# IlzeAmandaA/VAE-GP-ODE

Hardware: AMD Instinct MI355X
Metric: latent_trajectories_per_sec (higher is better)
Workload: dtype f32; 1 GPU; configs[1]: ode1 DF q=6 M=100 S=256 T=16 batch=256; step = full ELBO training step (encoder, GP draw, rk4 rollout, decoder, ELBO, backward, Adam), L=1; global_batch=256, mc_draws=1, solver=rk4 (3/8 rule), parallelism=dp1, hip_graph=True, graph_scope=whole, gp_side_stream=True, batchnorm=per-process statistics

## Files before the change

vae-gp-ode_amd/csrc/gp_backward.hip:

```cpp
#include "gp_rollout.hpp"

namespace gp {

template <int DI, int DO, int NJ>
__device__ __forceinline__ void store_grads_rbf(const typename RbfTeamEval<DI, DO, NJ>::Grads& G, float* __restrict__ out, int M, int S,
                                                int wave, int lane, float (*sInd)[64][4 * RbfLayout<DI, DO>::RQ2],
                                                float (*sUni)[((DO + 1) / 2) * DI]);
template <int D, int NJ, int PART = 0>
__device__ __forceinline__ void store_grads_df(const typename DfTeamEval<D, NJ>::Grads& G, float* __restrict__ out, int M, int S, int wave,
                                               int lane, float (*sInd)[64][4 * DfLayout<D>::RQ2],
                                               float (*sUni)[2 * D * ((D + 1) / 2) + (D + 1) / 2]);

template <class EV, bool PG> struct GradsOf { using type = NoGrads; };
template <class EV> struct GradsOf<EV, true> { using type = typename EV::Grads; };

template <class EV, int DI, int DO, int ORDER, int METHOD, bool PG = false, bool SUB = false>
__global__ __launch_bounds__(64 * EV::kTeam) void rollout_bwd_team_kernel(const float* __restrict__ pack, int M, int S,
                                                                const float* __restrict__ xstage, const float* __restrict__ gzt,
                                                                const float* __restrict__ ts, int N, int T,
                                                                float* __restrict__ gz0, float* __restrict__ astage, Draws dw,
                                                                float* __restrict__ slab = nullptr, size_t pack_floats = 0) {
  constexpr int NS = stages_of(METHOD);
  __shared__ float slots[2 * EV::kTeam * TeamCombine::DP];
  pack += blockIdx.y * dw.pack; xstage += blockIdx.y * dw.in; gzt += blockIdx.y * dw.in2; gz0 += blockIdx.y * dw.out; astage += blockIdx.y * dw.out2;
// ... 87 lines not shown
    } else {
      using L = DfLayout<DO>;
      constexpr int DH = (DO + 1) / 2;
      __shared__ __attribute__((aligned(16))) float sInd[2][64][4 * L::RQ2];
      __shared__ float sUni[TEAM][2 * DO * DH + DH];
      store_grads_df<DO, 1>(G, out, M, S, wave, lane, sInd, sUni);
    }
  }
}

template <class EV, int DI, int DO>
__global__ __launch_bounds__(64 * EV::kTeam) void rhs_vjp_team_kernel(const float* __restrict__ pack, int M, int S,
                                                            const float* __restrict__ x, const float* __restrict__ a, int R,
                                                            float* __restrict__ gx, int prior_only, Draws dw) {
  __shared__ float slots[2 * EV::kTeam * TeamCombine::DP];
  pack += blockIdx.y * dw.pack; x += blockIdx.y * dw.in; a += blockIdx.y * dw.in2; gx += blockIdx.y * dw.out;
  const int lane = threadIdx.x & 63, wave = threadIdx.x >> 6;
  EV ev;
  ev.init(pack, M, S, slots, wave, lane);
  for (int n = blockIdx.x; n < R; n += gridDim.x) {
    float xv[DI], av[DO], g[DI];
#pragma unroll
    for (int i = 0; i < DI; ++i) xv[i] = x[(size_t)n * DI + i];
#pragma unroll
    for (int i = 0; i < DO; ++i) av[i] = a[(size_t)n * DO + i];
    ev.vjp(xv, av, g, prior_only != 0);
    if (wave == 0) store_state<DI>(gx + (size_t)n * DI, g, lane);
  }
}

__device__ __forceinline__ void st4(float* __restrict__ base, size_t f4_index, const float* v) {
  reinterpret_cast<float4*>(base)[f4_index] = make_float4(v[0], v[1], v[2], v[3]);
}

template <int DI, int DO, int NJ>
__device__ __forceinline__ void store_grads_rbf(const typename RbfTeamEval<DI, DO, NJ>::Grads& G, float* __restrict__ out, int M, int S,
                                                int wave, int lane, float (*sInd)[64][4 * RbfLayout<DI, DO>::RQ2],
                                                float (*sUni)[((DO + 1) / 2) * DI]) {
  using L = RbfLayout<DI, DO>;
  constexpr int DH = (DO + 1) / 2;
  const int SJ = cdiv(S, 64), MJ = cdiv(M, 64);
#pragma unroll
  for (int jn = 0; jn < NJ; ++jn) {
    const int j = wave + TEAM * jn;
    if (j < SJ) {
#pragma unroll
      for (int d = 0; d < DO; ++d)
#pragma unroll
        for (int q = 0; q < L::RQ; ++q) st4(out, (size_t)((j * DO + d) * L::RQ + q) * 64 + lane, &G.rff[jn * DO + d][4 * q]);
    }
  }
  const int j = wave >> 1, half = wave & 1;
  if (half == 1) {
#pragma unroll
    for (int q = 0; q < 4 * L::RQ2; ++q) sInd[j][lane][q] = G.ind[q];
  }
  {
    float flat[DH * DI], red[DH * DI];
#pragma unroll
    for (int e = 0; e < DH * DI; ++e) flat[e] = G.gwl[e / DI][e % DI];
    wave_sum_all<DH * DI>(flat, red);
    if (lane == 0) {
#pragma unroll
      for (int e = 0; e < DH * DI; ++e) sUni[wave][e] = red[e];
    }
  }
  __syncthreads();
  if (half == 0 && j < MJ) {
    float* ind_out = out + 4 * L::rff_f4(S);
    float v[4 * L::RQ2];
#pragma unroll
    for (int q = 0; q < 4 * L::RQ2; ++q) v[q] = G.ind[q] + sInd[j][lane][q];
#pragma unroll
    for (int q = 0; q < L::RQ2; ++q) st4(ind_out, (size_t)(j * L::RQ2 + q) * 64 + lane, &v[4 * q]);
  }
  if (threadIdx.x < DO * DI) {
    const int d = threadIdx.x / DI, i = threadIdx.x % DI;
    const int h = d / DH, dd = d % DH;
    float* uni_out = out + 4 * (L::rff_f4(S) + L::ind_f4(M));
    uni_out[d * DI + i] = sUni[h][dd * DI + i] + sUni[h + 2][dd * DI + i];
  }
}

template <int DI, int DO, int NJ>
__global__ __launch_bounds__(256) void param_grad_rbf_kernel(const float* __restrict__ pack, int M, int S,
                                                              const float* __restrict__ xr, const float* __restrict__ ar,
                                                              int R, int rows_per_chunk, float* __restrict__ slab,
                                                              size_t pack_floats, int prior_only, Draws dw, int slab_chunks) {
  pack += blockIdx.y * dw.pack; xr += blockIdx.y * dw.in; ar += blockIdx.y * dw.in2; slab += (size_t)blockIdx.y * slab_chunks * pack_floats;
  using EV = RbfTeamEval<DI, DO, NJ>;
  using L = RbfLayout<DI, DO>;
  constexpr int DH = (DO + 1) / 2;
  __shared__ float slots[2 * TEAM * TeamCombine::DP];
  __shared__ __attribute__((aligned(16))) float sInd[2][64][4 * L::RQ2];
  __shared__ float sUni[TEAM][DH * DI];
  const int lane = threadIdx.x & 63, wave = threadIdx.x >> 6;
  EV ev;
  ev.init(pack, M, S, slots, wave, lane);
  typename EV::Grads G;
  G.zero();
  const int r0 = blockIdx.x * rows_per_chunk;
  const int r1 = min(R, r0 + rows_per_chunk);
  for (int r = r0; r < r1; ++r) {
    float x[DI], a[DO];
#pragma unroll
    for (int i = 0; i < DI; ++i) x[i] = xr[(size_t)r * DI + i];
#pragma unroll
    for (int i = 0; i < DO; ++i) a[i] = ar[(size_t)r * DO + i];
    ev.grad_row(x, a, G, prior_only != 0);
  }
  store_grads_rbf<DI, DO, NJ>(G, slab + (size_t)blockIdx.x * pack_floats, M, S, wave, lane, sInd, sUni);
}

template <int D, int NJ, int PART>
__device__ __forceinline__ void store_grads_df(const typename DfTeamEval<D, NJ>::Grads& G, float* __restrict__ out, int M, int S, int wave,
                                               int lane, float (*sInd)[64][4 * DfLayout<D>::RQ2],
                                               float (*sUni)[2 * D * ((D + 1) / 2) + (D + 1) / 2]) {
  using L = DfLayout<D>;
  constexpr int DH = (D + 1) / 2;
  constexpr int NU = 2 * D * DH + DH;
  const int SJ = cdiv(S, 64), MJ = cdiv(M, 64);
  if constexpr (PART != 2) {
#pragma unroll
    for (int jn = 0; jn < NJ; ++jn) {
      const int j = wave + TEAM * jn;
      if (j < SJ) {
#pragma unroll
        for (int i = 0; i < D; ++i)
#pragma unroll
          for (int q = 0; q < L::RQ; ++q) st4(out, (size_t)((j * D + i) * L::RQ + q) * 64 + lane, &G.rff[jn * D + i][4 * q]);
      }
    }
  }
  if constexpr (PART == 1) return;
  const int j = wave >> 1, half = wave & 1;
  if (half == 1) {
#pragma unroll
    for (int q = 0; q < 4 * L::RQ2; ++q) sInd[j][lane][q] = G.ind[q];
  }
  {
    float flat[NU];
#pragma unroll
    for (int a = 0; a < D; ++a)
#pragma unroll
      for (int b = 0; b < DH; ++b) { flat[a * DH + b] = G.gwab[a][b]; flat[D * DH + a * DH + b] = G.gil2[a][b]; }
#pragma unroll
    for (int b = 0; b < DH; ++b) flat[2 * D * DH + b] = G.gvar[b];
    float red[NU];
    wave_sum_all<NU>(flat, red);
    if (lane == 0) {
#pragma unroll
      for (int e = 0; e < NU; ++e) sUni[wave][e] = red[e];
    }
  }
  __syncthreads();
  if (half == 0 && j < MJ) {
    float* ind_out = out + 4 * L::rff_f4(S);
    float v[4 * L::RQ2];
#pragma unroll
    for (int q = 0; q < 4 * L::RQ2; ++q) v[q] = G.ind[q] + sInd[j][lane][q];
#pragma unroll
    for (int q = 0; q < L::RQ2; ++q) st4(ind_out, (size_t)(j * L::RQ2 + q) * 64 + lane, &v[4 * q]);
  }
  {
    float* uni_out = out + 4 * (L::rff_f4(S) + L::ind_f4(M));
    const int t = threadIdx.x;
    if (t < D * D) {
      const int a = t / D, b = t % D, h = b / DH, bb = b % DH;
      uni_out[a * D + b] = sUni[h][a * DH + bb] + sUni[h + 2][a * DH + bb];
      uni_out[D * D + a * D + b] = sUni[h][D * DH + a * DH + bb] + sUni[h + 2][D * DH + a * DH + bb];
    }
    if (t < D) {
      const int h = t / DH, bb = t % DH;
      uni_out[2 * D * D + t] = sUni[h][2 * D * DH + bb] + sUni[h + 2][2 * D * DH + bb];
    }
  }
}

template <int D, int NJ>
__global__ __launch_bounds__(256) void param_grad_df_kernel(const float* __restrict__ pack, int M, int S,
                                                             const float* __restrict__ xr, const float* __restrict__ ar,
                                                             int R, int rows_per_chunk, float* __restrict__ slab,
                                                             size_t pack_floats, int prior_only, Draws dw, int slab_chunks) {
  pack += blockIdx.y * dw.pack; xr += blockIdx.y * dw.in; ar += blockIdx.y * dw.in2; slab += (size_t)blockIdx.y * slab_chunks * pack_floats;
  using EV = DfTeamEval<D, NJ>;
  using L = DfLayout<D>;
  constexpr int DH = (D + 1) / 2;
  constexpr int NU = 2 * D * DH + DH;
  __shared__ float slots[2 * TEAM * TeamCombine::DP];
  __shared__ __attribute__((aligned(16))) float sInd[2][64][4 * L::RQ2];
  __shared__ float sUni[TEAM][NU];
  const int lane = threadIdx.x & 63, wave = threadIdx.x >> 6;
  EV ev;
  ev.init(pack, M, S, slots, wave, lane);
  typename EV::Grads G;
  G.zero();
  const int r0 = blockIdx.x * rows_per_chunk;
  const int r1 = min(R, r0 + rows_per_chunk);
  for (int r = r0; r < r1; ++r) {
    float x[D], a[D];
#pragma unroll
    for (int i = 0; i < D; ++i) { x[i] = xr[(size_t)r * D + i]; a[i] = ar[(size_t)r * D + i]; }
    ev.grad_row(x, a, G, prior_only != 0);
  }
  store_grads_df<D, NJ>(G, slab + (size_t)blockIdx.x * pack_floats, M, S, wave, lane, sInd, sUni);
}

template <int D, int PART>
__device__ __forceinline__ void pgrad_df_part(const float* __restrict__ pack, int M, int S, const float* __restrict__ xr,
                                              const float* __restrict__ ar, int r0, int r1, float* __restrict__ out, int prior_only) {
  using EV = DfTeamEval<D, 1>;
  using L = DfLayout<D>;
  constexpr int DH = (D + 1) / 2;
  constexpr int NU = 2 * D * DH + DH;
  __shared__ float slots[2 * TEAM * TeamCombine::DP];
  __shared__ __attribute__((aligned(16))) float sInd[2][64][4 * L::RQ2];
  __shared__ float sUni[TEAM][NU];
  const int lane = threadIdx.x & 63, wave = threadIdx.x >> 6;
  EV ev;
  ev.init(pack, M, S, slots, wave, lane);
  typename EV::Grads G;
  G.zero();
  for (int r = r0; r < r1; ++r) {
    float x[D], a[D];
#pragma unroll
    for (int i = 0; i < D; ++i) { x[i] = xr[(size_t)r * D + i]; a[i] = ar[(size_t)r * D + i]; }
    ev.template grad_row_part<PART>(x, a, G, prior_only != 0);
  }
  store_grads_df<D, 1, PART>(G, out, M, S, wave, lane, sInd, sUni);
}
template <int D>
__global__ __launch_bounds__(256, 2) void param_grad_df_split_kernel(const float* __restrict__ pack, int M, int S,
                                                                      const float* __restrict__ xr, const float* __restrict__ ar,
                                                                      int R, int rows_per_chunk, float* __restrict__ slab,
                                                                      size_t pack_floats, int prior_only, Draws dw, int slab_chunks) {
  pack += blockIdx.y * dw.pack; xr += blockIdx.y * dw.in; ar += blockIdx.y * dw.in2; slab += (size_t)blockIdx.y * slab_chunks * pack_floats;
  const int r0 = blockIdx.x * rows_per_chunk, r1 = min(R, r0 + rows_per_chunk);
  float* out = slab + (size_t)blockIdx.x * pack_floats;
  if (blockIdx.z == 0) pgrad_df_part<D, 1>(pack, M, S, xr, ar, r0, r1, out, prior_only);
  else pgrad_df_part<D, 2>(pack, M, S, xr, ar, r0, r1, out, prior_only);
}

template <int DI, int DO>
__global__ __launch_bounds__(256) void param_grad_rbf_stream_kernel(const float* __restrict__ pack, int M, int S,
                                                                     const float* __restrict__ xr, const float* __restrict__ ar,
                                                                     int R, int rows_per_chunk, float* __restrict__ slab,
                                                                     size_t pack_floats, int prior_only, Draws dw, int slab_chunks) {
  pack += blockIdx.y * dw.pack; xr += blockIdx.y * dw.in; ar += blockIdx.y * dw.in2; slab += (size_t)blockIdx.y * slab_chunks * pack_floats;
  using L = RbfLayout<DI, DO>;
  constexpr int DH = (DO + 1) / 2;
  __shared__ __attribute__((aligned(16))) float sInd[2][64][4 * L::RQ2];
  __shared__ float sUni[TEAM][DH * DI];
  const int lane = threadIdx.x & 63, wave = __builtin_amdgcn_readfirstlane(threadIdx.x >> 6);
  const float4* p4 = reinterpret_cast<const float4*>(pack);
  const float4* i4 = p4 + L::rff_f4(S);
  const float* wl = pack + 4 * (L::rff_f4(S) + L::ind_f4(M));
  const int r0 = blockIdx.x * rows_per_chunk, r1 = min(R, r0 + rows_per_chunk);
  float* out = slab + (size_t)blockIdx.x * pack_floats;
  const int SJ = cdiv(S, 64), MJ = cdiv(M, 64);
  for (int rec = wave; rec < SJ * DO; rec += TEAM) {
    float4 rq[L::RQ];
    load_record<L::RQ>(p4, rec, lane, rq);
    float g[4 * L::RQ];
#pragma unroll
    for (int q = 0; q < 4 * L::RQ; ++q) g[q] = 0.f;
    const int d = rec % DO;
    for (int r = r0; r < r1; ++r) {
      float x[DI], gx[DI];
#pragma unroll
      for (int i = 0; i < DI; ++i) { x[i] = xr[(size_t)r * DI + i]; gx[i] = 0.f; }
      rbf_rff_bwd<DI, DO, true>(rq, x, ar[(size_t)r * DO + d], gx, g);
    }
#pragma unroll
    for (int q = 0; q < L::RQ; ++q) st4(out, ((size_t)rec * L::RQ + q) * 64 + lane, &g[4 * q]);
  }
  const int half = wave & 1;
  float gwl[DH][DI];
#pragma unroll
  for (int d = 0; d < DH; ++d)
#pragma unroll
    for (int i = 0; i < DI; ++i) gwl[d][i] = 0.f;
  float* ind_out = out + 4 * L::rff_f4(S);
  for (int jb = 0; jb < MJ; jb += 2) {
    const int j = jb + (wave >> 1);
    const bool valid = j < MJ;
    float4 ind[L::RQ2];
    float gi[4 * L::RQ2];
#pragma unroll
    for (int q = 0; q < 4 * L::RQ2; ++q) gi[q] = 0.f;
    if (valid) {
      load_record<L::RQ2>(i4, j, lane, ind);
      if (!prior_only) {
        for (int r = r0; r < r1; ++r) {
          asm volatile("" ::: "memory");
          float x[DI], a[DO], gx[DI];
#pragma unroll
          for (int i = 0; i < DI; ++i) { x[i] = xr[(size_t)r * DI + i]; gx[i] = 0.f; }
#pragma unroll
          for (int i = 0; i < DO; ++i) a[i] = ar[(size_t)r * DO + i];
          rbf_ind_half_bwd<DI, DO, true>(ind, x, wl, half, a, gx, gi, gwl);
        }
      }
    }
    if (half == 1) {
#pragma unroll
      for (int q = 0; q < 4 * L::RQ2; ++q) sInd[wave >> 1][lane][q] = gi[q];
    }
    __syncthreads();
    if (half == 0 && valid) {
      float v[4 * L::RQ2];
#pragma unroll
// ... 306 lines not shown
```

vae-gp-ode_amd/csrc/gp_eval.hpp:

```cpp
#pragma once
#include <hip/hip_runtime.h>
#include "wave_reduce.hpp"

#define GP_WAVE 64
#define GP_LOG2E 1.4426950408889634f
#define GP_INV2PI 0.15915494309189535f

namespace gp {

__host__ __device__ constexpr int cdiv(int a, int b) { return (a + b - 1) / b; }

template <int DI, int DO> struct RbfLayout {
  static constexpr int RQ = cdiv(DI + 2, 4);
  static constexpr int RQ2 = cdiv(DI + DO, 4);
  __host__ __device__ static size_t rff_f4(int S) { return (size_t)cdiv(S, 64) * DO * RQ * 64; }
  __host__ __device__ static size_t ind_f4(int M) { return (size_t)cdiv(M, 64) * RQ2 * 64; }
  __host__ __device__ static size_t uni_floats() { return (size_t)cdiv(DO * DI, 4) * 4; }
  __host__ __device__ static size_t total_floats(int M, int S) { return 4 * (rff_f4(S) + ind_f4(M)) + uni_floats(); }
};

template <int D> struct DfLayout {
  static constexpr int RQ = cdiv(2 * D + 3, 4);
  static constexpr int RQ2 = cdiv(2 * D, 4);
  __host__ __device__ static size_t rff_f4(int S) { return (size_t)cdiv(S, 64) * D * RQ * 64; }
// ... 220 lines not shown
#pragma unroll
  for (int k = 0; k < D; ++k) t = fmaf(x[k], f[k], t);
  t = __builtin_amdgcn_fractf(t);
  const float c = __builtin_amdgcn_cosf(t), sn = __builtin_amdgcn_sinf(t);
  float A = 0.f;
#pragma unroll
  for (int j = 0; j < D; ++j) A = fmaf(a[j], f[D + 3 + j], A);
  const float rt = GP_2PI * fmaf(f[D + 2], c, -f[D + 1] * sn);
  const float coef = A * rt;
#pragma unroll
  for (int k = 0; k < D; ++k) gx[k] = fmaf(coef, f[k], gx[k]);
  if (WITH_G) {
    const float rr = fmaf(f[D + 2], sn, f[D + 1] * c);
#pragma unroll
    for (int k = 0; k < D; ++k) g[k] = fmaf(coef, x[k], g[k]);
#pragma unroll
    for (int j = 0; j < D; ++j) g[D + 3 + j] = fmaf(a[j], rr, g[D + 3 + j]);
  }
}

template <int D, bool WITH_G>
__device__ __forceinline__ void df_ind_half_bwd(const float4 (&r)[DfLayout<D>::RQ2], const float (&x)[D],
                                                const float* __restrict__ uni, int half, const float (&a)[D],
                                                float (&gx)[D], float (&g)[4 * DfLayout<D>::RQ2],
                                                float (&gwab)[D][(D + 1) / 2], float (&gil2)[D][(D + 1) / 2],
                                                float (&gvar)[(D + 1) / 2]) {
  constexpr int DH = (D + 1) / 2;
  float f[4 * DfLayout<D>::RQ2];
  unpack(r, f);
  const float* wab = uni;
  const float* il2 = uni + D * D;
  const float* var = uni + 2 * D * D;
  float dl[D];
  float r2 = 0.f;
#pragma unroll
  for (int q = 0; q < D; ++q) { dl[q] = x[q] - f[q]; r2 = fmaf(dl[q], dl[q], r2); }
  const int b0 = half * DH;
  float gd[D];
  float gr2 = 0.f;
#pragma unroll
  for (int q = 0; q < D; ++q) gd[q] = 0.f;
#pragma unroll
  for (int bb = 0; bb < DH; ++bb) {
    const bool hi_ok = DH + bb < D;
    const int bidx = b0 + bb < D ? b0 + bb : D - 1;
    const bool live = half ? hi_ok : true;
    const float dlb = half ? (hi_ok ? dl[hi_ok ? DH + bb : 0] : 0.f) : dl[bb];
    const float ab = live ? (half ? (hi_ok ? a[hi_ok ? DH + bb : 0] : 0.f) : a[bb]) : 0.f;
    const float vb = var[bidx];
    float gdb = 0.f;
    float gv = 0.f;
#pragma unroll
    for (int aa = 0; aa < D; ++aa) {
      const float il = il2[aa * D + bidx], wv = wab[aa * D + bidx];
      const float E = exp2_fast(r2 * wv);
      const bool diag = (aa == bidx);
      const float term = dl[aa] * dlb * il + (diag ? ((float)(D - 1) - r2 * il) : 0.f);
      const float G = ab * f[D + aa];
      const float GE = G * vb * E * il;
      gr2 = fmaf(GE, term * (GP_LN2 * wv) - (diag ? il : 0.f), gr2);
      gd[aa] = fmaf(GE * il, dlb, gd[aa]);
      gdb = fmaf(GE * il, dl[aa], gdb);
      if (WITH_G) {
        g[D + aa] = fmaf(ab, vb * E * il * term, g[D + aa]);
        gv = fmaf(G, E * il * term, gv);
        gwab[aa][bb] = fmaf(G * vb * il * term, E * GP_LN2 * r2, gwab[aa][bb]);
        gil2[aa][bb] = fmaf(G * vb * E, term + il * (dl[aa] * dlb - (diag ? r2 : 0.f)), gil2[aa][bb]);
      }
    }
    if (WITH_G) gvar[bb] += gv;
    if (live) {
      if (half) { if (hi_ok) gd[hi_ok ? DH + bb : 0] += gdb; }
      else gd[bb] += gdb;
    }
  }
#pragma unroll
  for (int q = 0; q < D; ++q) {
    const float v = fmaf(2.f * gr2, dl[q], gd[q]);
    gx[q] += v;
    if (WITH_G) g[q] -= v;
  }
}

template <int DI, int DO>
__device__ __forceinline__ void rbf_rff_jvp(const float4 (&r)[RbfLayout<DI, DO>::RQ], const float (&x)[DI], const float (&v)[DI],
                                            float& acc, float& jacc) {
  float f[4 * RbfLayout<DI, DO>::RQ];
  unpack(r, f);
  float t = f[DI], tv = 0.f;
#pragma unroll
  for (int i = 0; i < DI; ++i) { t = fmaf(x[i], f[i], t); tv = fmaf(v[i], f[i], tv); }
  t = __builtin_amdgcn_fractf(t);
  const float c = __builtin_amdgcn_cosf(t), sn = __builtin_amdgcn_sinf(t);
  acc = fmaf(f[DI + 1], c, acc);
  jacc = fmaf(f[DI + 1] * (-GP_2PI) * sn, tv, jacc);
}

template <int DI, int DO>
__device__ __forceinline__ void rbf_ind_jvp(const float4 (&r)[RbfLayout<DI, DO>::RQ2], const float (&x)[DI], const float (&v)[DI],
                                            const float* __restrict__ wl, float (&acc)[DO], float (&jacc)[DO]) {
  float f[4 * RbfLayout<DI, DO>::RQ2];
  unpack(r, f);
  float t2[DI], dt2[DI];
#pragma unroll
  for (int i = 0; i < DI; ++i) { const float d = x[i] - f[i]; t2[i] = d * d; dt2[i] = 2.f * d * v[i]; }
#pragma unroll
  for (int d = 0; d < DO; ++d) {
    float e = 0.f, de = 0.f;
#pragma unroll
    for (int i = 0; i < DI; ++i) { e = fmaf(wl[d * DI + i], t2[i], e); de = fmaf(wl[d * DI + i], dt2[i], de); }
    const float E = exp2_fast(e);
    acc[d] = fmaf(f[DI + d], E, acc[d]);
    jacc[d] = fmaf(f[DI + d] * E, GP_LN2 * de, jacc[d]);
  }
}

template <int D>
__device__ __forceinline__ void df_rff_jvp(const float4 (&r)[DfLayout<D>::RQ], const float (&x)[D], const float (&v)[D],
                                           float (&acc)[D], float (&jacc)[D]) {
  float f[4 * DfLayout<D>::RQ];
  unpack(r, f);
  float t = f[D], tv = 0.f;
#pragma unroll
  for (int k = 0; k < D; ++k) { t = fmaf(x[k], f[k], t); tv = fmaf(v[k], f[k], tv); }
  t = __builtin_amdgcn_fractf(t);
  const float c = __builtin_amdgcn_cosf(t), sn = __builtin_amdgcn_sinf(t);
  const float rr = fmaf(f[D + 2], sn, f[D + 1] * c);
  const float drr = GP_2PI * fmaf(f[D + 2], c, -f[D + 1] * sn) * tv;
#pragma unroll
  for (int j = 0; j < D; ++j) { acc[j] = fmaf(rr, f[D + 3 + j], acc[j]); jacc[j] = fmaf(drr, f[D + 3 + j], jacc[j]); }
}

template <int D>
__device__ __forceinline__ void df_ind_jvp(const float4 (&r)[DfLayout<D>::RQ2], const float (&x)[D], const float (&v)[D],
                                           const float* __restrict__ uni, float (&acc)[D], float (&jacc)[D]) {
  float f[4 * DfLayout<D>::RQ2];
  unpack(r, f);
  const float* wab = uni;
  const float* il2 = uni + D * D;
  const float* var = uni + 2 * D * D;
  float dl[D];
  float r2 = 0.f, dr2 = 0.f;
#pragma unroll
  for (int a = 0; a < D; ++a) { dl[a] = x[a] - f[a]; r2 = fmaf(dl[a], dl[a], r2); dr2 = fmaf(dl[a], v[a], dr2); }
  dr2 *= 2.f;
  if constexpr (D > 8) {
    constexpr int DH = (D + 1) / 2;
#pragma unroll 1
    for (int half = 0; half < 2; ++half) {
#pragma unroll
      for (int bb = 0; bb < DH; ++bb) {
        const bool valid = DH + bb < D;
        const int bidx = half * DH + bb < D ? half * DH + bb : D - 1;
        const float dlb = half ? (valid ? dl[valid ? DH + bb : 0] : 0.f) : dl[bb];
        const float vb = half ? (valid ? v[valid ? DH + bb : 0] : 0.f) : v[bb];
        float sb = 0.f, dsb = 0.f;
#pragma unroll
        for (int a = 0; a < D; ++a) {
          const float il = il2[a * D + bidx], wv = wab[a * D + bidx];
          const float E = exp2_fast(r2 * wv);
          const bool diag = (a == bidx);
          const float term = dl[a] * dlb * il + (diag ? ((float)(D - 1) - r2 * il) : 0.f);
          const float dterm = fmaf(v[a], dlb, dl[a] * vb) * il - (diag ? dr2 * il : 0.f);
          const float cf = f[D + a] * (E * il);
          sb = fmaf(cf, term, sb);
          dsb = fmaf(cf, fmaf(term, GP_LN2 * wv * dr2, dterm), dsb);
// ... 30 lines not shown
```

vae-gp-ode_amd/csrc/gp_team.hpp:

```cpp
#pragma once
#include "gp_eval.hpp"

namespace gp {

constexpr int TEAM = 4;

template <int TS> struct TeamCombineT {
  static constexpr int DP = 16;
  float* slots;
  int wave, lane, parity;
  __device__ __forceinline__ void init(float* s, int w, int l) { slots = s; wave = w; lane = l; parity = 0; }
  template <int NV> __device__ __forceinline__ void run(const float (&part)[NV], float (&f)[NV]) {
    static_assert(NV <= DP, "slot too small");
    float* mine = slots + (parity * TS + wave) * DP;
    if (lane == 0) {
#pragma unroll
      for (int d = 0; d < NV; ++d) mine[d] = part[d];
    }
    __syncthreads();
    const float* base = slots + parity * TS * DP;
#pragma unroll
    for (int d = 0; d < NV; ++d) {
      float v = base[d];
#pragma unroll
// ... 90 lines not shown
    for (int i = 0; i < DI; ++i) acc[i] = 0.f;
#pragma unroll
    for (int r = 0; r < NJ * DO; ++r) rbf_rff_bwd<DI, DO, true>(rff[r], x, a[r % DO], acc, G.rff[r]);
    rbf_ind_half_bwd<DI, DO, true>(ind, x, wl, half, a, acc, G.ind, G.gwl);
    float part[DI];
    wave_sum_all<DI>(acc, part);
    comb.run<DI>(part, gx);
  }
};

template <int D, int NJ> struct DfTeamEval {
  using L = DfLayout<D>;
  static constexpr int kTeam = TEAM;
  float4 rff[NJ * D][L::RQ];
  float4 ind[L::RQ2];
  const float* uni;
  int half;
  TeamCombine comb;
  static __host__ bool fits(int M, int S) { return cdiv(S, 64) <= TEAM * NJ && cdiv(M, 64) * 2 <= TEAM; }
  __device__ __forceinline__ void init(const float* pack, int M, int S, float* lds, int wave, int lane) {
    const float4* p4 = reinterpret_cast<const float4*>(pack);
    const int SJ = cdiv(S, 64), MJ = cdiv(M, 64);
    const float4 z = make_float4(0.f, 0.f, 0.f, 0.f);
#pragma unroll
    for (int jn = 0; jn < NJ; ++jn) {
      const int j = wave + TEAM * jn;
#pragma unroll
      for (int i = 0; i < D; ++i)
#pragma unroll
        for (int q = 0; q < L::RQ; ++q) rff[jn * D + i][q] = j < SJ ? p4[((j * D + i) * L::RQ + q) * 64 + lane] : z;
    }
    const float4* i4 = p4 + L::rff_f4(S);
    const int j = wave >> 1;
    half = wave & 1;
#pragma unroll
    for (int q = 0; q < L::RQ2; ++q) ind[q] = j < MJ ? i4[(j * L::RQ2 + q) * 64 + lane] : z;
    uni = pack + 4 * (L::rff_f4(S) + L::ind_f4(M));
    comb.init(lds, wave, lane);
  }
  template <int MODE> __device__ __forceinline__ void eval(const float (&x)[D], float (&f)[D]) {
    float acc[D];
#pragma unroll
    for (int d = 0; d < D; ++d) acc[d] = 0.f;
    if (MODE != 2) {
#pragma unroll
      for (int r = 0; r < NJ * D; ++r) df_rff_record<D>(rff[r], x, acc);
    }
    if (MODE != 1) df_ind_record_half<D>(ind, x, uni, half, acc);
    float part[D];
    wave_sum_all<D>(acc, part);
    comb.run<D>(part, f);
  }
  __device__ __forceinline__ void vjp(const float (&x)[D], const float (&a)[D], float (&gx)[D], bool prior_only = false) {
    float acc[D];
#pragma unroll
    for (int i = 0; i < D; ++i) acc[i] = 0.f;
    float g0[4 * L::RQ], g1[4 * L::RQ2], g2[D][(D + 1) / 2], g3[D][(D + 1) / 2], g4[(D + 1) / 2];
#pragma unroll
    for (int r = 0; r < NJ * D; ++r) df_rff_bwd<D, false>(rff[r], x, a, acc, g0);
    if (!prior_only) df_ind_half_bwd<D, false>(ind, x, uni, half, a, acc, g1, g2, g3, g4);
    float part[D];
    wave_sum_all<D>(acc, part);
    comb.run<D>(part, gx);
  }
  struct Grads {
    float rff[NJ * D][4 * L::RQ];
    float ind[4 * L::RQ2];
    float gwab[D][(D + 1) / 2], gil2[D][(D + 1) / 2], gvar[(D + 1) / 2];
    __device__ __forceinline__ void zero() {
#pragma unroll
      for (int r = 0; r < NJ * D; ++r)
#pragma unroll
        for (int q = 0; q < 4 * L::RQ; ++q) rff[r][q] = 0.f;
#pragma unroll
      for (int q = 0; q < 4 * L::RQ2; ++q) ind[q] = 0.f;
#pragma unroll
      for (int a = 0; a < D; ++a)
#pragma unroll
        for (int b = 0; b < (D + 1) / 2; ++b) { gwab[a][b] = 0.f; gil2[a][b] = 0.f; }
#pragma unroll
      for (int b = 0; b < (D + 1) / 2; ++b) gvar[b] = 0.f;
    }
  };
  __device__ __forceinline__ void grad_row(const float (&x)[D], const float (&a)[D], Grads& G, bool prior_only) const {
    float gx[D];
#pragma unroll
    for (int i = 0; i < D; ++i) gx[i] = 0.f;
#pragma unroll
    for (int r = 0; r < NJ * D; ++r) df_rff_bwd<D, true>(rff[r], x, a, gx, G.rff[r]);
    if (!prior_only) df_ind_half_bwd<D, true>(ind, x, uni, half, a, gx, G.ind, G.gwab, G.gil2, G.gvar);
  }
  template <int PART> __device__ __forceinline__ void grad_row_part(const float (&x)[D], const float (&a)[D], Grads& G, bool prior_only) const {
    float gx[D];
#pragma unroll
    for (int i = 0; i < D; ++i) gx[i] = 0.f;
    if constexpr (PART != 2) {
#pragma unroll
      for (int r = 0; r < NJ * D; ++r) df_rff_bwd<D, true>(rff[r], x, a, gx, G.rff[r]);
    }
    if constexpr (PART != 1) {
      if (!prior_only) df_ind_half_bwd<D, true>(ind, x, uni, half, a, gx, G.ind, G.gwab, G.gil2, G.gvar);
    }
  }
  __device__ __forceinline__ void vjp_grad(const float (&x)[D], const float (&a)[D], float (&gx)[D], Grads& G) {
    float acc[D];
#pragma unroll
    for (int i = 0; i < D; ++i) acc[i] = 0.f;
#pragma unroll
    for (int r = 0; r < NJ * D; ++r) df_rff_bwd<D, true>(rff[r], x, a, acc, G.rff[r]);
    df_ind_half_bwd<D, true>(ind, x, uni, half, a, acc, G.ind, G.gwab, G.gil2, G.gvar);
    float part[D];
    wave_sum_all<D>(acc, part);
    comb.run<D>(part, gx);
  }
};

template <int NQ>
__device__ __forceinline__ void load_record(const float4* __restrict__ base, int rec, int lane, float4 (&r)[NQ]) {
#pragma unroll
  for (int q = 0; q < NQ; ++q) r[q] = base[((size_t)rec * NQ + q) * 64 + lane];
}

template <int N> __device__ __forceinline__ float pick(const float (&v)[N], int idx) {
  float r = v[0];
#pragma unroll
  for (int i = 1; i < N; ++i) r = (idx == i) ? v[i] : r;
  return r;
}

template <int D, int NP, bool WITH_G>
__device__ __forceinline__ void df_ind_part_bwd(const float4 (&r)[DfLayout<D>::RQ2], const float (&x)[D],
                                                const float* __restrict__ uni, int part, const float (&a)[D],
                                                float (&gx)[D], float (&g)[4 * DfLayout<D>::RQ2],
                                                float (&gwab)[D][(D + NP - 1) / NP], float (&gil2)[D][(D + NP - 1) / NP],
                                                float (&gvar)[(D + NP - 1) / NP]) {
  constexpr int DQ = (D + NP - 1) / NP;
  float f[4 * DfLayout<D>::RQ2];
  unpack(r, f);
  const float* wab = uni;
  const float* il2 = uni + D * D;
  const float* var = uni + 2 * D * D;
  float dl[D];
  float r2 = 0.f;
#pragma unroll
  for (int q = 0; q < D; ++q) { dl[q] = x[q] - f[q]; r2 = fmaf(dl[q], dl[q], r2); }
  float gd[D];
  float gr2 = 0.f;
#pragma unroll
  for (int q = 0; q < D; ++q) gd[q] = 0.f;
#pragma unroll
  for (int bb = 0; bb < DQ; ++bb) {
    const int b = part * DQ + bb;
    const bool live = b < D;
    const int bidx = live ? b : D - 1;
    const float dlb = live ? pick<D>(dl, bidx) : 0.f;
    const float ab = live ? pick<D>(a, bidx) : 0.f;
    const float vb = var[bidx];
    float gdb = 0.f, gv = 0.f;
#pragma unroll
    for (int aa = 0; aa < D; ++aa) {
      const float il = il2[aa * D + bidx], wv = wab[aa * D + bidx];
      const float E = exp2_fast(r2 * wv);
      const bool diag = (aa == bidx);
      const float term = dl[aa] * dlb * il + (diag ? ((float)(D - 1) - r2 * il) : 0.f);
      const float G = ab * f[D + aa];
      const float GE = G * vb * E * il;
      gr2 = fmaf(GE, term * (GP_LN2 * wv) - (diag ? il : 0.f), gr2);
      gd[aa] = fmaf(GE * il, dlb, gd[aa]);
      gdb = fmaf(GE * il, dl[aa], gdb);
      if (WITH_G) {
        g[D + aa] = fmaf(ab, vb * E * il * term, g[D + aa]);
        gv = fmaf(G, E * il * term, gv);
        gwab[aa][bb] = fmaf(G * vb * il * term, E * GP_LN2 * r2, gwab[aa][bb]);
        gil2[aa][bb] = fmaf(G * vb * E, term + il * (dl[aa] * dlb - (diag ? r2 : 0.f)), gil2[aa][bb]);
      }
    }
    if (WITH_G) gvar[bb] += gv;
#pragma unroll
    for (int q = 0; q < D; ++q) gd[q] += (live && q == bidx) ? gdb : 0.f;
  }
#pragma unroll
  for (int q = 0; q < D; ++q) {
    const float v = fmaf(2.f * gr2, dl[q], gd[q]);
    gx[q] += v;
    if (WITH_G) g[q] -= v;
// ... 140 lines not shown
```

vae-gp-ode_amd/csrc/vae_dense.hip:

```cpp
#include <hip/hip_runtime.h>
#include "gp_launch.hpp"
#include "wave_reduce.hpp"

namespace gp {

__global__ void k_act_fwd(const float* __restrict__ x, float* __restrict__ y, size_t n, int mode) {
  for (size_t e = (size_t)blockIdx.x * blockDim.x + threadIdx.x; e < n; e += (size_t)gridDim.x * blockDim.x) {
    const float v = x[e];
    y[e] = mode == 0 ? fmaxf(v, 0.f) : 1.f / (1.f + expf(-v));
  }
}
__global__ void k_act_bwd(const float* __restrict__ y, const float* __restrict__ gy, float* __restrict__ gx, size_t n, int mode) {
  for (size_t e = (size_t)blockIdx.x * blockDim.x + threadIdx.x; e < n; e += (size_t)gridDim.x * blockDim.x) {
    const float v = y[e];
    gx[e] = mode == 0 ? (v > 0.f ? gy[e] : 0.f) : gy[e] * v * (1.f - v);
  }
}

__global__ void k_linear_fwd(const float* __restrict__ x, const float* __restrict__ w, const float* __restrict__ bias,
                             float* __restrict__ y, int B, int In, int Out) {
  const size_t e = (size_t)blockIdx.x * blockDim.x + threadIdx.x;
  if (e >= (size_t)B * Out) return;
  const int b = (int)(e / Out), o = (int)(e % Out);
  float acc = bias ? bias[o] : 0.f;
  const float* xr = x + (size_t)b * In;
  const float* wr = w + (size_t)o * In;
  for (int i = 0; i < In; ++i) acc = fmaf(xr[i], wr[i], acc);
  y[e] = acc;
}
__global__ void k_linear_bwd_x(const float* __restrict__ gy, const float* __restrict__ w, float* __restrict__ gx, int B, int In, int Out,
                               const float* __restrict__ xpre) {
  const size_t e = (size_t)blockIdx.x * blockDim.x + threadIdx.x;
  if (e >= (size_t)B * In) return;
  const int b = (int)(e / In), i = (int)(e % In);
  float acc = 0.f;
  for (int o = 0; o < Out; ++o) acc = fmaf(gy[(size_t)b * Out + o], w[(size_t)o * In + i], acc);
  gx[e] = (xpre && !(xpre[e] > 0.f)) ? 0.f : acc;
}
__global__ __launch_bounds__(256) void k_linear_bwd_w(const float* __restrict__ x, const float* __restrict__ gy, float* __restrict__ gw,
                                                       float* __restrict__ gb, int B, int In, int Out, int relu_in) {
  const int wave = (blockIdx.x * blockDim.x + threadIdx.x) >> 6, lane = threadIdx.x & 63;
  if (wave >= Out * (In + 1)) return;
  const int o = wave / (In + 1), i = wave % (In + 1);
  if (i < In ? !gw : !gb) return;
  float acc = 0.f;
  for (int b = lane; b < B; b += 64) {
    float xv = i < In ? x[(size_t)b * In + i] : 1.f;
    if (relu_in && i < In) xv = fmaxf(xv, 0.f);
    acc = fmaf(gy[(size_t)b * Out + o], xv, acc);
  }
  float in1[1] = {acc}, out1[1];
  wave_sum_multi<1>(in1, out1);
  if (lane == 0) { if (i < In) gw[(size_t)o * In + i] = out1[0]; else gb[o] = out1[0]; }
}

constexpr int LINW_SLABS = 32;
__global__ __launch_bounds__(256) void k_linear_bwd_w_cols(const float* __restrict__ x, const float* __restrict__ gy, float* __restrict__ partW,
                                                            float* __restrict__ partB, int B, int In, int Out, int rps) {
  __shared__ float red[4][9][64];
  const int lane = threadIdx.x & 63, g = threadIdx.x >> 6, o = blockIdx.x * 64 + lane;
  const int b0 = blockIdx.y * rps, b1 = min(B, b0 + rps);
  float acc[9];
#pragma unroll
  for (int i = 0; i < 9; ++i) acc[i] = 0.f;
#pragma unroll 4
  for (int b = b0 + g; b < b1; b += 4) {
    const float gv = gy[(size_t)b * Out + o];
    const float* xr = x + (size_t)b * In;
#pragma unroll
    for (int i = 0; i < 8; ++i)
      if (i < In) acc[i] = fmaf(gv, xr[i], acc[i]);
    acc[8] += gv;
  }
#pragma unroll
  for (int i = 0; i < 9; ++i) red[g][i][lane] = acc[i];
  __syncthreads();
  for (int e = threadIdx.x; e < 9 * 64; e += 256) {
    const int i = e >> 6, l = e & 63, oo = blockIdx.x * 64 + l;
    const float v = (red[0][i][l] + red[1][i][l]) + (red[2][i][l] + red[3][i][l]);
    if (i < In) partW[((size_t)blockIdx.y * Out + oo) * In + i] = v;
    else if (i == 8) partB[(size_t)blockIdx.y * Out + oo] = v;
  }
}

__global__ __launch_bounds__(256) void k_linear_fwd_fanin(const float* __restrict__ x, const float* __restrict__ w,
                                                           const float* __restrict__ bias, float* __restrict__ y, int B, int In, int Out,
                                                           int relu_in) {
  const int lane = threadIdx.x & 63;
  const int e = blockIdx.x * 4 + (threadIdx.x >> 6);
  if (e >= B * Out) return;
  const int b = e / Out, o = e % Out;
  const float* xr = x + (size_t)b * In;
  const float* wr = w + (size_t)o * In;
  float acc = 0.f;
  if (relu_in) { for (int i = lane; i < In; i += 64) acc = fmaf(fmaxf(xr[i], 0.f), wr[i], acc); }
  else { for (int i = lane; i < In; i += 64) acc = fmaf(xr[i], wr[i], acc); }
  const float in1[1] = {acc};
  float out1[1];
  wave_sum_multi<1>(in1, out1);
  if (lane == 0) y[e] = out1[0] + (bias ? bias[o] : 0.f);
}

constexpr int LIN_MAXIN = 16;
__global__ __launch_bounds__(256) void k_linear_fwd_fanout(const float* __restrict__ x, const float* __restrict__ w,
                                                            const float* __restrict__ bias, float* __restrict__ y, int B, int In, int Out,
                                                            int rows_per_block) {
  const int b0 = blockIdx.x * rows_per_block, b1 = min(B, b0 + rows_per_block);
  for (int o = blockIdx.y * 256 + threadIdx.x; o < Out; o += 256 * gridDim.y) {
    float wr[LIN_MAXIN];
#pragma unroll
    for (int i = 0; i < LIN_MAXIN; ++i) wr[i] = i < In ? w[(size_t)o * In + i] : 0.f;
    const float bo = bias ? bias[o] : 0.f;
    for (int b = b0; b < b1; ++b) {
      const float* xr = x + (size_t)b * In;
      float acc = bo;
#pragma unroll
      for (int i = 0; i < LIN_MAXIN; ++i)
        if (i < In) acc = fmaf(xr[i], wr[i], acc);
      y[(size_t)b * Out + o] = acc;
    }
  }
}
template <int OPL>
__global__ __launch_bounds__(256) void k_linear_bwd_x_fanout(const float* __restrict__ gy, const float* __restrict__ w, float* __restrict__ gx,
                                                              int B, int In) {
  const int lane = threadIdx.x & 63, wave = threadIdx.x >> 6, nw = gridDim.x * 4;
  constexpr int Out = OPL * 64;
  float wr[OPL][LIN_MAXIN];
#pragma unroll
  for (int k = 0; k < OPL; ++k)
#pragma unroll
    for (int i = 0; i < LIN_MAXIN; ++i) wr[k][i] = i < In ? w[(size_t)(lane + 64 * k) * In + i] : 0.f;
  for (int b = blockIdx.x * 4 + wave; b < B; b += nw) {
    float acc[LIN_MAXIN];
#pragma unroll
    for (int i = 0; i < LIN_MAXIN; ++i) acc[i] = 0.f;
#pragma unroll
    for (int k = 0; k < OPL; ++k) {
      const float g = gy[(size_t)b * Out + lane + 64 * k];
#pragma unroll
      for (int i = 0; i < LIN_MAXIN; ++i) acc[i] = fmaf(g, wr[k][i], acc[i]);
    }
    float tot[LIN_MAXIN];
    wave_sum_all<LIN_MAXIN>(acc, tot);
    if (lane < In) {
      float v = 0.f;
#pragma unroll
      for (int i = 0; i < LIN_MAXIN; ++i) v = (lane == i) ? tot[i] : v;
      gx[(size_t)b * In + lane] = v;
    }
  }
}

int act_fwd(const float* x, float* y, size_t n, int mode, hipStream_t st) {
  hipLaunchKernelGGL(k_act_fwd, ew_grid(n), 256, 0, st, x, y, n, mode);
// ... 68 lines not shown
```

Before: 108,700 trajectories/s.

## Prefetch GP grad rows, cache DF tail params in registers, tile linear-bwd inputs in LDS

The DF parameter-gradient kernels now prefetch the next row's x/a one iteration ahead and specialize the prior_only flag at compile time. The per-half inducing-tail hyperparameters (wab, il2, var) are loaded once into registers instead of being re-read from the uniform pack on every row. Separately, the linear-layer weight-gradient kernel stages input rows in shared memory per 128-row tile and batches its gy loads. The changes are meant to hide global-load latency and cut redundant loads, at the cost of extra registers, which may lower occupancy.

```diff
diff --git a/vae-gp-ode_amd/csrc/gp_backward.hip b/vae-gp-ode_amd/csrc/gp_backward.hip
--- a/vae-gp-ode_amd/csrc/gp_backward.hip
+++ b/vae-gp-ode_amd/csrc/gp_backward.hip
@@ -193,6 +193,37 @@
   }
 }
 
+template <int DI, int DO, class ROW>
+__device__ __forceinline__ void chunk_rows_ahead(const float* __restrict__ xr, const float* __restrict__ ar, int r0, int r1, ROW&& row) {
+  if (r0 >= r1) return;
+  float xn[DI], an[DO];
+#pragma unroll
+  for (int i = 0; i < DI; ++i) xn[i] = __int_as_float(__builtin_amdgcn_readfirstlane(__float_as_int(xr[(size_t)r0 * DI + i])));
+#pragma unroll
+  for (int i = 0; i < DO; ++i) an[i] = __int_as_float(__builtin_amdgcn_readfirstlane(__float_as_int(ar[(size_t)r0 * DO + i])));
+  __builtin_amdgcn_s_waitcnt(0x0070);
+  for (int r = r0; r < r1; ++r) {
+    float x[DI], a[DO];
+#pragma unroll
+    for (int i = 0; i < DI; ++i) x[i] = xn[i];
+#pragma unroll
+    for (int i = 0; i < DO; ++i) a[i] = an[i];
+    const int rn = min(r + 1, r1 - 1);
+#pragma unroll
+    for (int i = 0; i < DI; ++i) xn[i] = xr[(size_t)rn * DI + i];
+#pragma unroll
+    for (int i = 0; i < DO; ++i) an[i] = ar[(size_t)rn * DO + i];
+    __builtin_amdgcn_sched_barrier(0);
+    row(x, a);
+  }
+}
+template <int DI, int DO, class ROW>
+__device__ __forceinline__ void chunk_rows_ahead(const float* __restrict__ xr, const float* __restrict__ ar, int r0, int r1, int prior_only,
+                                                 ROW&& row) {
+  if (prior_only) chunk_rows_ahead<DI, DO>(xr, ar, r0, r1, [&](const float (&x)[DI], const float (&a)[DO]) { row(x, a, std::true_type()); });
+  else chunk_rows_ahead<DI, DO>(xr, ar, r0, r1, [&](const float (&x)[DI], const float (&a)[DO]) { row(x, a, std::false_type()); });
+}
+
 template <int DI, int DO, int NJ>
 __global__ __launch_bounds__(256) void param_grad_rbf_kernel(const float* __restrict__ pack, int M, int S,
                                                               const float* __restrict__ xr, const float* __restrict__ ar,
@@ -304,16 +335,14 @@
   const int lane = threadIdx.x & 63, wave = threadIdx.x >> 6;
   EV ev;
   ev.init(pack, M, S, slots, wave, lane);
+  typename EV::Tail tail;
+  ev.load_tail(tail, __builtin_amdgcn_readfirstlane(threadIdx.x >> 6) & 1);
   typename EV::Grads G;
   G.zero();
   const int r0 = blockIdx.x * rows_per_chunk;
   const int r1 = min(R, r0 + rows_per_chunk);
-  for (int r = r0; r < r1; ++r) {
-    float x[D], a[D];
-#pragma unroll
-    for (int i = 0; i < D; ++i) { x[i] = xr[(size_t)r * D + i]; a[i] = ar[(size_t)r * D + i]; }
-    ev.grad_row(x, a, G, prior_only != 0);
-  }
+  chunk_rows_ahead<D, D>(xr, ar, r0, r1, prior_only,
+                         [&](const float (&x)[D], const float (&a)[D], auto po) { ev.grad_row(x, a, G, decltype(po)::value, tail); });
   store_grads_df<D, NJ>(G, slab + (size_t)blockIdx.x * pack_floats, M, S, wave, lane, sInd, sUni);
 }
 
@@ -330,14 +359,16 @@
   const int lane = threadIdx.x & 63, wave = threadIdx.x >> 6;
   EV ev;
   ev.init(pack, M, S, slots, wave, lane);
+  typename EV::Tail tail;
+  if constexpr (PART != 1) ev.load_tail(tail, __builtin_amdgcn_readfirstlane(threadIdx.x >> 6) & 1);
   typename EV::Grads G;
   G.zero();
-  for (int r = r0; r < r1; ++r) {
-    float x[D], a[D];
-#pragma unroll
-    for (int i = 0; i < D; ++i) { x[i] = xr[(size_t)r * D + i]; a[i] = ar[(size_t)r * D + i]; }
-    ev.template grad_row_part<PART>(x, a, G, prior_only != 0);
-  }
+  if constexpr (PART == 1)
+    chunk_rows_ahead<D, D>(xr, ar, r0, r1, [&](const float (&x)[D], const float (&a)[D]) { ev.template grad_row_part<1>(x, a, G, false, tail); });
+  else
+    chunk_rows_ahead<D, D>(xr, ar, r0, r1, prior_only, [&](const float (&x)[D], const float (&a)[D], auto po) {
+      ev.template grad_row_part<PART>(x, a, G, decltype(po)::value, tail);
+    });
   store_grads_df<D, 1, PART>(G, out, M, S, wave, lane, sInd, sUni);
 }
 template <int D>
diff --git a/vae-gp-ode_amd/csrc/gp_eval.hpp b/vae-gp-ode_amd/csrc/gp_eval.hpp
--- a/vae-gp-ode_amd/csrc/gp_eval.hpp
+++ b/vae-gp-ode_amd/csrc/gp_eval.hpp
@@ -326,6 +326,79 @@
   }
 }
 
+template <int D> struct DfTailHalf {
+  static constexpr int DH = (D + 1) / 2;
+  float wab[D][DH], il2[D][DH], var[DH];
+  __device__ __forceinline__ void load(const float* __restrict__ uni, int half) {
+#pragma unroll
+    for (int bb = 0; bb < DH; ++bb) {
+      const int bidx = half * DH + bb < D ? half * DH + bb : D - 1;
+#pragma unroll
+      for (int aa = 0; aa < D; ++aa) { wab[aa][bb] = uni[aa * D + bidx]; il2[aa][bb] = uni[D * D + aa * D + bidx]; }
+      var[bb] = uni[2 * D * D + bidx];
+    }
+  }
+};
+
+template <int D, bool WITH_G>
+__device__ __forceinline__ void df_ind_half_bwd_t(const float4 (&r)[DfLayout<D>::RQ2], const float (&x)[D],
+                                                  const DfTailHalf<D>& tl, int half, const float (&a)[D],
+                                                  float (&gx)[D], float (&g)[4 * DfLayout<D>::RQ2],
+                                                  float (&gwab)[D][(D + 1) / 2], float (&gil2)[D][(D + 1) / 2],
+                                                  float (&gvar)[(D + 1) / 2]) {
+  constexpr int DH = (D + 1) / 2;
+  float f[4 * DfLayout<D>::RQ2];
+  unpack(r, f);
+  float dl[D];
+  float r2 = 0.f;
+#pragma unroll
+  for (int q = 0; q < D; ++q) { dl[q] = x[q] - f[q]; r2 = fmaf(dl[q], dl[q], r2); }
+  const int b0 = half * DH;
+  float gd[D];
+  float gr2 = 0.f;
+#pragma unroll
+  for (int q = 0; q < D; ++q) gd[q] = 0.f;
+#pragma unroll
+  for (int bb = 0; bb < DH; ++bb) {
+    const bool hi_ok = DH + bb < D;
+    const int bidx = b0 + bb < D ? b0 + bb : D - 1;
+    const bool live = half ? hi_ok : true;
+    const float dlb = half ? (hi_ok ? dl[hi_ok ? DH + bb : 0] : 0.f) : dl[bb];
+    const float ab = live ? (half ? (hi_ok ? a[hi_ok ? DH + bb : 0] : 0.f) : a[bb]) : 0.f;
+    const float vb = tl.var[bb];
+    float gdb = 0.f;
+    float gv = 0.f;
+#pragma unroll
+    for (int aa = 0; aa < D; ++aa) {
+      const float il = tl.il2[aa][bb], wv = tl.wab[aa][bb];
+      const float E = exp2_fast(r2 * wv);
+      const bool diag = (aa == bidx);
+      const float term = dl[aa] * dlb * il + (diag ? ((float)(D - 1) - r2 * il) : 0.f);
+      const float G = ab * f[D + aa];
+      const float GE = G * vb * E * il;
+      gr2 = fmaf(GE, term * (GP_LN2 * wv) - (diag ? il : 0.f), gr2);
+      gd[aa] = fmaf(GE * il, dlb, gd[aa]);
+      gdb = fmaf(GE * il, dl[aa], gdb);
+      if (WITH_G) {
+        g[D + aa] = fmaf(ab, vb * E * il * term, g[D + aa]);
+        gv = fmaf(G, E * il * term, gv);
+        gwab[aa][bb] = fmaf(G * vb * il * term, E * GP_LN2 * r2, gwab[aa][bb]);
+        gil2[aa][bb] = fmaf(G * vb * E, term + il * (dl[aa] * dlb - (diag ? r2 : 0.f)), gil2[aa][bb]);
+      }
+    }
+    if (WITH_G) gvar[bb] += gv;
+    if (live) {
+      if (half) { if (hi_ok) gd[hi_ok ? DH + bb : 0] += gdb; }
+      else gd[bb] += gdb;
+    }
+  }
+#pragma unroll
+  for (int q = 0; q < D; ++q) {
+    const float v = fmaf(2.f * gr2, dl[q], gd[q]);
+    gx[q] += v;
+    if (WITH_G) g[q] -= v;
+  }
+}
 template <int DI, int DO>
 __device__ __forceinline__ void rbf_rff_jvp(const float4 (&r)[RbfLayout<DI, DO>::RQ], const float (&x)[DI], const float (&v)[DI],
                                             float& acc, float& jacc) {
diff --git a/vae-gp-ode_amd/csrc/gp_team.hpp b/vae-gp-ode_amd/csrc/gp_team.hpp
--- a/vae-gp-ode_amd/csrc/gp_team.hpp
+++ b/vae-gp-ode_amd/csrc/gp_team.hpp
@@ -196,15 +196,10 @@
       for (int b = 0; b < (D + 1) / 2; ++b) gvar[b] = 0.f;
     }
   };
-  __device__ __forceinline__ void grad_row(const float (&x)[D], const float (&a)[D], Grads& G, bool prior_only) const {
-    float gx[D];
-#pragma unroll
-    for (int i = 0; i < D; ++i) gx[i] = 0.f;
-#pragma unroll
-    for (int r = 0; r < NJ * D; ++r) df_rff_bwd<D, true>(rff[r], x, a, gx, G.rff[r]);
-    if (!prior_only) df_ind_half_bwd<D, true>(ind, x, uni, half, a, gx, G.ind, G.gwab, G.gil2, G.gvar);
-  }
-  template <int PART> __device__ __forceinline__ void grad_row_part(const float (&x)[D], const float (&a)[D], Grads& G, bool prior_only) const {
+  using Tail = DfTailHalf<D>;
+  __device__ __forceinline__ void load_tail(Tail& tl, int half_uniform) const { tl.load(uni, half_uniform); }
+  template <int PART> __device__ __forceinline__ void grad_row_part(const float (&x)[D], const float (&a)[D], Grads& G, bool prior_only,
+                                                                    const Tail& tl) const {
     float gx[D];
 #pragma unroll
     for (int i = 0; i < D; ++i) gx[i] = 0.f;
@@ -213,8 +208,11 @@
       for (int r = 0; r < NJ * D; ++r) df_rff_bwd<D, true>(rff[r], x, a, gx, G.rff[r]);
     }
     if constexpr (PART != 1) {
-      if (!prior_only) df_ind_half_bwd<D, true>(ind, x, uni, half, a, gx, G.ind, G.gwab, G.gil2, G.gvar);
-    }
+      if (!prior_only) df_ind_half_bwd_t<D, true>(ind, x, tl, half, a, gx, G.ind, G.gwab, G.gil2, G.gvar);
+    }
+  }
+  __device__ __forceinline__ void grad_row(const float (&x)[D], const float (&a)[D], Grads& G, bool prior_only, const Tail& tl) const {
+    grad_row_part<0>(x, a, G, prior_only, tl);
   }
   __device__ __forceinline__ void vjp_grad(const float (&x)[D], const float (&a)[D], float (&gx)[D], Grads& G) {
     float acc[D];
diff --git a/vae-gp-ode_amd/csrc/vae_dense.hip b/vae-gp-ode_amd/csrc/vae_dense.hip
--- a/vae-gp-ode_amd/csrc/vae_dense.hip
+++ b/vae-gp-ode_amd/csrc/vae_dense.hip
@@ -55,22 +55,35 @@
 }
 
 constexpr int LINW_SLABS = 32;
+constexpr int LINW_TILE = 128;
 __global__ __launch_bounds__(256) void k_linear_bwd_w_cols(const float* __restrict__ x, const float* __restrict__ gy, float* __restrict__ partW,
                                                             float* __restrict__ partB, int B, int In, int Out, int rps) {
   __shared__ float red[4][9][64];
+  __shared__ float xs[LINW_TILE * 8];
   const int lane = threadIdx.x & 63, g = threadIdx.x >> 6, o = blockIdx.x * 64 + lane;
   const int b0 = blockIdx.y * rps, b1 = min(B, b0 + rps);
   float acc[9];
 #pragma unroll
   for (int i = 0; i < 9; ++i) acc[i] = 0.f;
-#pragma unroll 4
-  for (int b = b0 + g; b < b1; b += 4) {
-    const float gv = gy[(size_t)b * Out + o];
-    const float* xr = x + (size_t)b * In;
-#pragma unroll
-    for (int i = 0; i < 8; ++i)
-      if (i < In) acc[i] = fmaf(gv, xr[i], acc[i]);
-    acc[8] += gv;
+  for (int t0 = b0; t0 < b1; t0 += LINW_TILE) {
+    const int nr = min(LINW_TILE, b1 - t0);
+    float gv[LINW_TILE / 4];
+#pragma unroll
+    for (int k = 0; k < LINW_TILE / 4; ++k) gv[k] = gy[(size_t)(t0 + min(g + 4 * k, nr - 1)) * Out + o];
+    if (t0 != b0) __syncthreads();
+    for (int e = threadIdx.x; e < nr * In; e += 256) xs[e] = x[(size_t)t0 * In + e];
+    __syncthreads();
+#pragma unroll
+    for (int k = 0; k < LINW_TILE / 4; ++k) {
+      const int r = g + 4 * k;
+      if (r < nr) {
+        const float* xr = xs + r * In;
+#pragma unroll
+        for (int i = 0; i < 8; ++i)
+          if (i < In) acc[i] = fmaf(gv[k], xr[i], acc[i]);
+        acc[8] += gv[k];
+      }
+    }
   }
 #pragma unroll
   for (int i = 0; i < 9; ++i) red[g][i][lane] = acc[i];
```

New measurement: 109,900 trajectories/s, median of 6. 1.1% higher.
